# hjsuh94/irs_mpc

Measured on AMD Instinct MI355X. Metric: rollouts*timesteps/s (randomized-smoothing pass) + iLQR-iters/s, higher is better.
Workload: dtype f32; 1 GPU; planar_hand quasi-dynamic contact, zero-order-B smoothing, step QP solved exactly (dual active-set method) -- the metric's config; T=50, N_per_gpu=10000, N_total=10000, mode=ZERO_ORDER_B, contact_solver=exact, samples=supplied, resident in HBM (f32), parallelism=samples sharded over 1 GPU(s), 1 all-reduce of (T,P) f64 per step

## Files before the change

irs_mpc_amd/csrc/smooth_ug.hip:

```cpp
#include "smooth_common.hpp"

namespace {

#ifndef IRS_UG_SWEEPS
#define IRS_UG_SWEEPS 6
#endif
#ifndef IRS_UG_PDAS
#define IRS_UG_PDAS 4
#endif
#ifndef IRS_UG_BLOCK
#define IRS_UG_BLOCK 512
#endif
constexpr int kUgBlock = IRS_UG_BLOCK;
constexpr int kUgSweeps = IRS_UG_SWEEPS;
constexpr int kUgPdas = IRS_UG_PDAS;
#ifndef IRS_UG_STEP_COLUMNS
#define IRS_UG_STEP_COLUMNS 1
#endif
constexpr bool kUgStepColumns = IRS_UG_STEP_COLUMNS != 0;
constexpr int kUgTabH = 8, kUgTabTau = 40, kUgTabSet = 48, kUgTabX = 52;
constexpr int kUgTabStride = 116;
#ifndef IRS_UG_NOM_ROUNDS
#define IRS_UG_NOM_ROUNDS 2
#endif
constexpr int kUgNomRounds = IRS_UG_NOM_ROUNDS;
constexpr int kUgRing = 128;

template <class Model>
struct alignas(16) UgLds {
    static constexpr int NC = Model::NC, n = Model::NX, m = Model::NU;
    float tab[1 << NC][kUgTabStride];
    float W[NC][NC];
    float invw[NC];
    float Wd[NC];
    float r0[NC];
    float phi[NC];
    float C[m][NC];
    float JD[n][NC];
    float Jc[NC][n];
    float Dinv[n];
    float Db0[n];
    float DK[m];
    float q[n];
};

__device__ __forceinline__ float ug_uniform(float v) {
    return __int_as_float(__builtin_amdgcn_readfirstlane(__float_as_int(v)));
}

template <int NC>
struct UgUni {
    float W[NC * (NC + 1) / 2];
    float invw[NC];
    float r0[NC];
    __device__ __forceinline__ float w(int i, int j) const {
        return i <= j ? W[i * NC - i * (i - 1) / 2 + (j - i)] : W[j * NC - j * (j - 1) / 2 + (i - j)];
    }
};

template <class Model>
__device__ __forceinline__ unsigned ug_lookup_affine(const UgLds<Model>& S, unsigned a, const float* du, float tol,
                                                     float* v, float* tau) {
    constexpr int NC = Model::NC, m = Model::NU;
    static_assert(NC == 8 && m == 4, "table entries are 8 rows by 4 commands");
    const float4* e = reinterpret_cast<const float4*>(&S.tab[a][0]);
    float4 g4[kUgTabSet / 4];
#pragma unroll
    for (int c = 0; c < kUgTabSet / 4; ++c) g4[c] = e[c];
    const unsigned ap = __float_as_uint(S.tab[a][kUgTabSet]);
    tau[0] = g4[kUgTabTau / 4].x; tau[1] = g4[kUgTabTau / 4].y; tau[2] = g4[kUgTabTau / 4].z; tau[3] = g4[kUgTabTau / 4].w;
    tau[4] = g4[kUgTabTau / 4 + 1].x; tau[5] = g4[kUgTabTau / 4 + 1].y; tau[6] = g4[kUgTabTau / 4 + 1].z; tau[7] = g4[kUgTabTau / 4 + 1].w;
    v[0] = fmaf(tau[0], tol, g4[0].x); v[1] = fmaf(tau[1], tol, g4[0].y);
    v[2] = fmaf(tau[2], tol, g4[0].z); v[3] = fmaf(tau[3], tol, g4[0].w);
    v[4] = fmaf(tau[4], tol, g4[1].x); v[5] = fmaf(tau[5], tol, g4[1].y);
    v[6] = fmaf(tau[6], tol, g4[1].z); v[7] = fmaf(tau[7], tol, g4[1].w);
#pragma unroll
    for (int j = 0; j < m; ++j) {
        const float4 lo = g4[kUgTabH / 4 + 2 * j], hi = g4[kUgTabH / 4 + 2 * j + 1];
        v[0] = fmaf(lo.x, du[j], v[0]); v[1] = fmaf(lo.y, du[j], v[1]);
        v[2] = fmaf(lo.z, du[j], v[2]); v[3] = fmaf(lo.w, du[j], v[3]);
        v[4] = fmaf(hi.x, du[j], v[4]); v[5] = fmaf(hi.y, du[j], v[5]);
        v[6] = fmaf(hi.z, du[j], v[6]); v[7] = fmaf(hi.w, du[j], v[7]);
    }
    return ap;
}

template <class Model, bool UCOL>
__device__ __forceinline__ void ug_step_direction(const UgLds<Model>& S, unsigned a, int p, float* u, float* tau) {
    constexpr int NC = Model::NC;
    const float* e = &S.tab[a][0];
    const float4 t0 = *reinterpret_cast<const float4*>(e + kUgTabTau), t1 = *reinterpret_cast<const float4*>(e + kUgTabTau + 4);
    if constexpr (UCOL) {
        const float4 lo = *reinterpret_cast<const float4*>(e + kUgTabX + NC * p);
        const float4 hi = *reinterpret_cast<const float4*>(e + kUgTabX + NC * p + 4);
        u[0] = lo.x; u[1] = lo.y; u[2] = lo.z; u[3] = lo.w;
        u[4] = hi.x; u[5] = hi.y; u[6] = hi.z; u[7] = hi.w;
    } else {
        const float4 wlo = *reinterpret_cast<const float4*>(&S.W[p][0]);
        const float4 whi = *reinterpret_cast<const float4*>(&S.W[p][4]);
        const float4* x4 = reinterpret_cast<const float4*>(e + kUgTabX);
        float4 g4[2 * NC];
#pragma unroll
        for (int c = 0; c < 2 * NC; ++c) g4[c] = x4[c];
        const float wp[NC] = {wlo.x, wlo.y, wlo.z, wlo.w, whi.x, whi.y, whi.z, whi.w};
#pragma unroll
        for (int i = 0; i < NC; ++i) u[i] = 0.f;
#pragma unroll
        for (int c = 0; c < NC; ++c) {
            const float4 lo = g4[2 * c], hi = g4[2 * c + 1];
            u[0] = fmaf(lo.x, wp[c], u[0]); u[1] = fmaf(lo.y, wp[c], u[1]);
            u[2] = fmaf(lo.z, wp[c], u[2]); u[3] = fmaf(lo.w, wp[c], u[3]);
            u[4] = fmaf(hi.x, wp[c], u[4]); u[5] = fmaf(hi.y, wp[c], u[5]);
            u[6] = fmaf(hi.z, wp[c], u[6]); u[7] = fmaf(hi.w, wp[c], u[7]);
        }
    }
    tau[0] = t0.x; tau[1] = t0.y; tau[2] = t0.z; tau[3] = t0.w;
    tau[4] = t1.x; tau[5] = t1.y; tau[6] = t1.z; tau[7] = t1.w;
}

template <class Model>
__device__ __forceinline__ float ug_rhs(const UgUni<Model::NC>& U, const UgLds<Model>& S, const float* du, float* r) {
    constexpr int NC = Model::NC, m = Model::NU;
#pragma unroll
    for (int c = 0; c < NC; ++c) r[c] = U.r0[c];
#pragma unroll
    for (int j = 0; j < m; ++j) {
        const float4 lo = *reinterpret_cast<const float4*>(&S.C[j][0]);
        const float4 hi = *reinterpret_cast<const float4*>(&S.C[j][4]);
        r[0] = fmaf(lo.x, du[j], r[0]); r[1] = fmaf(lo.y, du[j], r[1]);
        r[2] = fmaf(lo.z, du[j], r[2]); r[3] = fmaf(lo.w, du[j], r[3]);
        r[4] = fmaf(hi.x, du[j], r[4]); r[5] = fmaf(hi.y, du[j], r[5]);
        r[6] = fmaf(hi.z, du[j], r[6]); r[7] = fmaf(hi.w, du[j], r[7]);
    }
    float scale = 1e-30f;
#pragma unroll
    for (int c = 0; c < NC; ++c) scale = fmaxf(scale, fabsf(r[c]));
    return 1e-6f * scale;
}

template <class Model>
__device__ __forceinline__ bool ug_try(const UgUni<Model::NC>& U, const UgLds<Model>& S, const float* r, const float* du,
                                       float tolv, float* lam, unsigned& a_out, int diag = 0) {
    constexpr int NC = Model::NC;
    float g[NC];
#pragma unroll
    for (int i = 0; i < NC; ++i) { lam[i] = 0.f; g[i] = r[i]; }
#pragma unroll 2
    for (int sw = 0; sw < ((diag & 64) ? 0 : kUgSweeps); ++sw) {
#pragma unroll
        for (int i = 0; i < NC; ++i) {
            const float nw = fmaxf(fmaf(-g[i], U.invw[i], lam[i]), 0.f);
            const float dl = nw - lam[i];
            lam[i] = nw;
#pragma unroll
            for (int j = 0; j < NC; ++j) g[j] = fmaf(U.w(j, i), dl, g[j]);
        }
    }
    unsigned a = 0u;
#pragma unroll
    for (int i = 0; i < NC; ++i) a |= (lam[i] > 0.f) ? (1u << i) : 0u;
    bool done = (diag & 32) != 0;
    for (int it = 0; it < kUgPdas; ++it) {
        float v[NC], tau[NC];
        const unsigned ap = ug_lookup_affine<Model>(S, a, du, tolv, v, tau);
        unsigned bad = 0u;
#pragma unroll
        for (int i = NC - 1; i >= 0; --i) bad = __builtin_amdgcn_alignbit(bad, __float_as_uint(v[i]), 31);
        if (!done) {
            if (bad == 0u) {
#pragma unroll
                for (int i = 0; i < NC; ++i) lam[i] = fmaf(-tau[i], v[i], v[i]);
                done = true;
            }
            a = ap ^ bad;
        }
        if (__all(done)) break;
    }
    a_out = a;
    return done;
}

template <class Model, bool UCOL>
__device__ __forceinline__ void ug_full(const UgLds<Model>& S, const float* r, const float* du, float tolv, unsigned a,
                                        float* lam, int cap = 4 * Model::NC) {
    constexpr int NC = Model::NC;
    constexpr float kBig = 3.0e38f, piv_rel = 1e-5f;
    float g[NC];
    bool valid = false;
    for (int round = 0; round < 3; ++round) {
        if (__all(valid)) break;
        float v[NC], tau[NC];
        const unsigned ap = ug_lookup_affine<Model>(S, a, du, 0.f, v, tau);
        if (!valid) {
            unsigned negb = 0u;
#pragma unroll
            for (int i = 0; i < NC; ++i) {
                const bool in = tau[i] == 0.f;
                negb |= (in && !(v[i] > 0.f)) ? (1u << i) : 0u;
                lam[i] = in ? v[i] : 0.f;
                g[i] = in ? 0.f : v[i];
            }
            valid = negb == 0u;
            a = ap & ~negb;
        }
    }
    if (!valid) {
        a = 0u;
#pragma unroll
        for (int i = 0; i < NC; ++i) { lam[i] = 0.f; g[i] = r[i]; }
    }
    int p = -1;
    bool done = false;
    for (int it = 0; it < cap; ++it) {
        if (!done && p < 0) {
            float vmin = kBig;
            int c = 0;
#pragma unroll
            for (int i = 0; i < NC; ++i) {
                const float vv = ((a >> i) & 1u) ? kBig : g[i];
                if (vv < vmin) { vmin = vv; c = i; }
            }
            if (vmin >= -tolv) done = true;
            else p = c;
        }
        if (__all(done)) break;
        const int pp = (done || p < 0) ? 0 : p;
        float u[NC], tau[NC];
        ug_step_direction<Model, UCOL>(S, a, pp, u, tau);
        const float wpp = S.Wd[pp];
        float gp = 0.f, zp = 0.f;
#pragma unroll
        for (int i = 0; i < NC; ++i) {
            const bool isp = i == pp;
            gp = isp ? g[i] : gp;
            zp = isp ? u[i] : zp;
        }
        const bool full_ok = zp > piv_rel * wpp;
        const float t2 = full_ok ? -gp * irs_rcp_fast(zp) : kBig;
        float rho[NC], qv[NC];
        float t1 = kBig;
#pragma unroll
        for (int i = 0; i < NC; ++i) {
            rho[i] = fmaf(tau[i], u[i], -u[i]);
            qv[i] = rho[i] > 0.f ? lam[i] * irs_rcp_fast(rho[i]) : kBig;
            t1 = fminf(t1, qv[i]);
        }
        int kb = 0;
#pragma unroll
        for (int i = NC - 1; i >= 0; --i) kb = (qv[i] == t1) ? i : kb;
        const float tmin = fminf(t1, t2);
        if (!done && !(tmin < kBig)) done = true;
        const float tt = done ? 0.f : tmin;
#pragma unroll
        for (int i = 0; i < NC; ++i) {
            g[i] = fmaf(tt * tau[i], u[i], g[i]);
            lam[i] = fmaxf(fmaf(-tt, rho[i], lam[i]) + ((i == pp) ? tt : 0.f), 0.f);
        }
        if (!done) {
            const bool full = t2 <= t1;
            if (full) {
                a |= 1u << pp;
                p = -1;
            } else {
                a &= ~(1u << kb);
#pragma unroll
                for (int i = 0; i < NC; ++i) lam[i] = (i == kb) ? 0.f : lam[i];
            }
        }
    }
}

template <class Model, bool UCOL>
__device__ __forceinline__ void ug_build_entry(UgLds<Model>& S, unsigned a, int half) {
    constexpr int NC = Model::NC;
    constexpr float piv_rel = 1e-5f;
    float M_[NC][NC], inv[NC], W[NC][NC];
    bool act[NC];
#pragma unroll
    for (int i = 0; i < NC; ++i) {
        act[i] = ((a >> i) & 1u) != 0u;
#pragma unroll
        for (int j = 0; j < NC; ++j) W[i][j] = S.W[i][j];
#pragma unroll
        for (int j = 0; j <= i; ++j) M_[i][j] = W[i][j];
    }
    unsigned ap = 0u;
#pragma unroll
    for (int j = 0; j < NC; ++j) {
        const float dj = M_[j][j];
        const bool ok = act[j] && dj > piv_rel * W[j][j];
        act[j] = ok;
        ap |= ok ? (1u << j) : 0u;
        inv[j] = ok ? irs_rcp_fast(dj) : 0.f;
#pragma unroll
        for (int i = j + 1; i < NC; ++i) M_[j][i] = M_[i][j] * inv[j];
#pragma unroll
        for (int i = j + 1; i < NC; ++i)
#pragma unroll
            for (int k = j + 1; k <= i; ++k) M_[i][k] = M_[i][k] - M_[j][i] * M_[k][j];
    }
    float* e = &S.tab[a][0];
    constexpr int NAPP = 1 + Model::NU + NC, SHARE = (NAPP + 1) / 2;
    for (int qq = 0; qq < SHARE; ++qq) {
        const int q = half * SHARE + qq;
        if (q >= NAPP) break;
        const int c = q - (1 + Model::NU);
        float x[NC];
        if (UCOL || c < 0) {
            const float* src = q == 0 ? &S.r0[0] : (c < 0 ? &S.C[q - 1][0] : &S.W[c][0]);
            const float4 lo = *reinterpret_cast<const float4*>(src), hi = *reinterpret_cast<const float4*>(src + 4);
            x[0] = lo.x; x[1] = lo.y; x[2] = lo.z; x[3] = lo.w;
            x[4] = hi.x; x[5] = hi.y; x[6] = hi.z; x[7] = hi.w;
        } else {
#pragma unroll
            for (int i = 0; i < NC; ++i) x[i] = (i == c) ? 1.f : 0.f;
        }
        float y[NC];
#pragma unroll
        for (int j = 0; j < NC; ++j) {
            float v = act[j] ? -x[j] : 0.f;
#pragma unroll
            for (int k = 0; k < j; ++k) v = v - M_[k][j] * y[k];
            y[j] = v;
        }
#pragma unroll
        for (int j = NC - 1; j >= 0; --j) {
            float v = y[j] * inv[j];
#pragma unroll
            for (int i = j + 1; i < NC; ++i) v = v - M_[j][i] * y[i];
            y[j] = v;
        }
        float col[NC];
#pragma unroll
        for (int i = 0; i < NC; ++i) {
            float s = x[i];
#pragma unroll
            for (int j = 0; j < NC; ++j) s = fmaf(W[i][j], y[j], s);
            col[i] = act[i] ? y[i] : s;
        }
        float* dst = e + (c < 0 ? NC * q : kUgTabX + NC * c);
        *reinterpret_cast<float4*>(dst) = make_float4(col[0], col[1], col[2], col[3]);
        *reinterpret_cast<float4*>(dst + 4) = make_float4(col[4], col[5], col[6], col[7]);
    }
    if (half == 1) {
        *reinterpret_cast<float4*>(e + kUgTabTau) = make_float4(act[0] ? 0.f : 1.f, act[1] ? 0.f : 1.f, act[2] ? 0.f : 1.f, act[3] ? 0.f : 1.f);
        *reinterpret_cast<float4*>(e + kUgTabTau + 4) = make_float4(act[4] ? 0.f : 1.f, act[5] ? 0.f : 1.f, act[6] ? 0.f : 1.f, act[7] ? 0.f : 1.f);
        e[kUgTabSet] = __uint_as_float(ap);
    }
}

struct UgNomLds {
    double J[8][7];
    double q[7], Dinv[7], b[7];
};

template <class Model, class Args>
__device__ __forceinline__ double ug_nominal_geometry(const Args& a, UgNomLds& L, int t, int lane) {
    constexpr int NC = Model::NC, n = Model::NX, m = Model::NU;
    double x64[n], u64[m], q[n], Dinv[n], b[n], J[NC][n], phi[NC];
#pragma unroll
    for (int i = 0; i < n; ++i) x64[i] = a.x_trj[(size_t)t * n + i];
#pragma unroll
    for (int j = 0; j < m; ++j) u64[j] = a.u_trj[(size_t)t * m + j];
    Model::template assemble<double>(a.p, x64, u64, q, Dinv, b, J, phi);
    if (lane == 0) {
#pragma unroll
        for (int c = 0; c < NC; ++c)
#pragma unroll
            for (int k = 0; k < n; ++k) L.J[c][k] = J[c][k];
#pragma unroll
        for (int k = 0; k < n; ++k) { L.q[k] = q[k]; L.Dinv[k] = Dinv[k]; L.b[k] = b[k]; }
    }
    double rr = 0.0;
#pragma unroll
    for (int c = 0; c < NC; ++c) {
        double s = phi[c];
#pragma unroll
        for (int k = 0; k < n; ++k) s -= J[c][k] * (b[k] * Dinv[k]);
        rr = (lane == c) ? s : rr;
    }
    wave_sync();
    return rr;
}

template <class Model, bool UCOL, class Args>
__device__ __forceinline__ void ug_nominal(const Args& a, const UgUni<Model::NC>& U, const UgLds<Model>& S,
                                           UgNomLds& L, double rr, int t, int lane) {
    constexpr int NC = Model::NC, n = Model::NX, m = Model::NU;
    static_assert(NC == 8 && n <= 8, "lane (i,k) = 8 i + k owns entry (i,k) of the 8 x 8 dual Hessian");
    float du0[m], r32[NC], lam32[NC];
#pragma unroll
    for (int j = 0; j < m; ++j) du0[j] = 0.f;
    const float tolv = ug_rhs<Model>(U, S, du0, r32);
    unsigned am = 0u;
    if (!ug_try<Model>(U, S, r32, du0, tolv, lam32, am)) ug_full<Model, UCOL>(S, r32, du0, tolv, am, lam32);
    unsigned set = 0u;
#pragma unroll
    for (int i = 0; i < NC; ++i) set |= (lam32[i] > 0.f) ? (1u << i) : 0u;
    set = (unsigned)__builtin_amdgcn_readfirstlane((int)set);
    {
        const int li = lane >> 3, lk = lane & 7;
        double w = 0.0;
#pragma unroll
        for (int kk = 0; kk < n; ++kk) w += L.J[li][kk] * L.Dinv[kk] * L.J[lk][kk];
        double scale = 1e-300;
#pragma unroll
        for (int c = 0; c < NC; ++c) scale = fmax(scale, fabs(__shfl(rr, c, 64)));
        const double tol64 = 1e-10 * scale;
        double lamd = 0.0;
        bool settled = false;
        for (int corr = 0; corr < 8 && !settled; ++corr) {
            double M = w, Lf = 0.0;
            unsigned eff = 0u;
            double invd[NC];
#pragma unroll
            for (int j = 0; j < NC; ++j) {
                const double dj = __shfl(M, 9 * j, 64), wjj = __shfl(w, 9 * j, 64);
                const bool ok = ((set >> j) & 1u) && dj > 1e-7 * wjj;
                eff |= ok ? (1u << j) : 0u;
                invd[j] = ok ? 1.0 / dj : 0.0;
                const double Mij = __shfl(M, 8 * li + j, 64), Mkj = __shfl(M, 8 * lk + j, 64);
                if (lk == j && li > j) Lf = Mij * invd[j];
                if (li > j && lk > j) M -= Mij * invd[j] * Mkj;
            }
            const bool mine = lane < NC && ((eff >> lane) & 1u);
            double y = mine ? -rr : 0.0;
#pragma unroll
            for (int j = 0; j < NC; ++j) {
                const double yj = __shfl(y, j, 64);
                const double Lij = __shfl(Lf, 8 * (lane & 7) + j, 64);
                if (lane < NC && lane > j) y -= Lij * yj;
            }
            double invme = 0.0;
#pragma unroll
            for (int j = 0; j < NC; ++j) invme = (lane == j) ? invd[j] : invme;
            y *= invme;
#pragma unroll
            for (int j = NC - 1; j >= 0; --j) {
                const double yj = __shfl(y, j, 64);
                const double Lji = __shfl(Lf, 8 * j + (lane & 7), 64);
                if (lane < j) y -= Lji * yj;
            }
            lamd = mine ? y : 0.0;
            double pr = w * __shfl(lamd, lk, 64);
            pr += __shfl_xor(pr, 1, 64);
            pr += __shfl_xor(pr, 2, 64);
            pr += __shfl_xor(pr, 4, 64);
            const double sl = rr + __shfl(pr, 8 * (lane & 7), 64);
            const bool neg = lane < NC && mine && !(lamd > 0.0);
            const bool viol = lane < NC && !mine && sl < -tol64;
            const unsigned negb = (unsigned)(__ballot(neg) & 0xffull), violb = (unsigned)(__ballot(viol) & 0xffull);
            if ((negb | violb) == 0u) settled = true;
            else set = (eff & ~negb) | violb;
        }
        double f = 0.0;
        if (settled) {
            double acc = 0.0;
#pragma unroll
            for (int c = 0; c < NC; ++c) acc += L.J[c][lane < n ? lane : 0] * __shfl(lamd, c, 64);
            if (lane < n) f = L.q[lane] + L.Dinv[lane] * (acc - L.b[lane]);
        } else if (lane < n) {
            float acc = -S.Db0[lane];
#pragma unroll
            for (int c = 0; c < NC; ++c) acc = fmaf(S.JD[lane][c], lam32[c], acc);
            f = (double)(S.q[lane] + acc);
        }
        if (lane < n)
            __hip_atomic_store(a.fnom + (size_t)t * n + Model::perm(lane), f, __ATOMIC_RELAXED, __HIP_MEMORY_SCOPE_AGENT);
    }
}

#ifdef IRS_UG_STAMPS
constexpr int kUgStampSlots = 12, kUgStampWgs = 2048;
__device__ unsigned long long ug_stamps[kUgStampWgs * kUgStampSlots];
#define UG_STAMP(slot)                                                                          \
    do {                                                                                        \
        if ((threadIdx.x & 63) == 0) {                                                          \
            const int wg_ = blockIdx.y * gridDim.x + blockIdx.x;                                \
            if (wg_ < kUgStampWgs && ((slot) < 8 ? threadIdx.x == 0 : true))                    \
                ug_stamps[wg_ * kUgStampSlots + (slot)] = __builtin_amdgcn_s_memtime();         \
        }                                                                                       \
    } while (0)
#else
#define UG_STAMP(slot) do {} while (0)
#endif

template <class Model, int MODE, bool RNG, bool FUSE, bool BATCH>
__global__ __launch_bounds__(kUgBlock) void smooth_ug_kernel(SmoothArgs args, std::conditional_t<BATCH, SmoothBatch, SmoothSolo> bat) {
    using TR = SmoothTraits<Model, MODE>;
    constexpr int n = TR::n, m = TR::m, P = TR::P, NC = Model::NC;
    constexpr int BLOCK = kUgBlock, NW = BLOCK / 64;
    static_assert(TR::Z0 == n && NC == 8 && m == 4, "u-only smoothing of an 8-row contact model with 4 commands");
    static_assert(P < kBlock, "the hand-off's group reduction");
    constexpr int NG = m * (m + 1) / 2;
    constexpr int PI = TR::FIRST_B ? 1 : NG + m * NC + m;
    constexpr int PPI = irs_reduce_pad(TR::FIRST_B ? n * m : PI);
    constexpr int QE = m + 1;
    constexpr bool UCOL = !TR::FIRST_B && kUgStepColumns;
    __shared__ UgLds<Model> S;
    __shared__ UgNomLds nomL;
    __shared__ float ring_all[NW * kUgRing * QE];
    __shared__ float red[NW * (PPI > TR::PP ? PPI : TR::PP)];
    __shared__ float toti[PPI];
    __shared__ unsigned hist[TR::FIRST_B ? (1 << NC) : 1];
    __shared__ double red64[TR::NGRP * P];
    __shared__ double tot[P];
    __shared__ FinalizeLds<Model, MODE> fin;
    __shared__ int s_ticket;

    decltype(auto) a = smooth_row<Model, MODE>(args, bat, (int)blockIdx.y);
    const int t = smooth_row_t(a, (int)blockIdx.y), blk = blockIdx.x, tid = threadIdx.x;
    const int lane = tid & 63, wave = tid >> 6;

    UG_STAMP(0);
    const bool nominal_wave = blk == 0 && wave == NW - 1;
    double nom_r = 0.0;
    if (nominal_wave && !(a.diag & 2)) nom_r = ug_nominal_geometry<Model>(a, nomL, t, lane);
    if (wave == 0) {
        float xb[n], ub[m], q[n], Dinv[n], b0[n], J[NC][n], phi[NC];
#pragma unroll
        for (int i = 0; i < n; ++i) xb[i] = (float)a.x_trj[(size_t)t * n + i];
#pragma unroll
        for (int j = 0; j < m; ++j) ub[j] = (float)a.u_trj[(size_t)t * m + j];
        Model::template assemble<float>(a.p, xb, ub, q, Dinv, b0, J, phi);
        if (lane == 0) {
#pragma unroll
            for (int i = 0; i < NC; ++i) {
                S.phi[i] = phi[i];
#pragma unroll
                for (int k = 0; k < n; ++k) S.Jc[i][k] = J[i][k];
            }
#pragma unroll
            for (int k = 0; k < n; ++k) { S.Db0[k] = b0[k] * Dinv[k]; S.q[k] = q[k]; S.Dinv[k] = Dinv[k]; }
#pragma unroll
            for (int j = 0; j < m; ++j) S.DK[j] = Dinv[Model::act(j)] * Model::template stiffness<float>(a.p, j);
        }
    }
    if constexpr (TR::FIRST_B) {
        for (int q = tid; q < (1 << NC); q += BLOCK) hist[q] = 0u;
    }
    __syncthreads();
    if (tid < NC * NC) {
        const int i = tid / NC, j = tid % NC, hi = i > j ? i : j, lo = i > j ? j : i;
        float w = (S.Jc[hi][0] * S.Dinv[0]) * S.Jc[lo][0];
#pragma unroll
        for (int k = 1; k < n; ++k) w = w + (S.Jc[hi][k] * S.Dinv[k]) * S.Jc[lo][k];
        S.W[i][j] = w;
        if (i == j) {
            S.Wd[i] = w;
            S.invw[i] = (float)kContactPgsOmega * irs_rcp_fast(w);
        }
    } else if (tid < NC * NC + NC) {
        const int i = tid - NC * NC;
        float ri = S.phi[i];
#pragma unroll
        for (int k = 0; k < n; ++k) ri = ri - S.Jc[i][k] * S.Db0[k];
        S.r0[i] = ri;
    } else if (tid < 2 * NC * NC + NC) {
        const int e = tid - (NC * NC + NC), k = e / NC, c = e % NC;
        if (k < n) S.JD[k][c] = S.Jc[c][k] * S.Dinv[k];
    } else if (tid < 2 * NC * NC + NC + m * NC) {
        const int e = tid - (2 * NC * NC + NC), j = e / NC, c = e % NC;
        S.C[j][c] = (S.Jc[c][Model::act(j)] * S.Dinv[Model::act(j)]) * Model::template stiffness<float>(a.p, j);
    }
    __syncthreads();
    UG_STAMP(1);
    if (!(a.diag & 4))
        for (int e = tid; e < 2 * (1 << NC); e += BLOCK) ug_build_entry<Model, UCOL>(S, (unsigned)(e >> 1), e & 1);
    __syncthreads();

    UG_STAMP(2);
    UgUni<NC> U;
    {
        int q = 0;
#pragma unroll
        for (int i = 0; i < NC; ++i)
#pragma unroll
            for (int j = i; j < NC; ++j) U.W[q++] = S.W[i][j];
#pragma unroll
        for (int i = 0; i < NC; ++i) { U.invw[i] = S.invw[i]; U.r0[i] = S.r0[i]; }
    }

    float acc[PPI];
#pragma unroll
    for (int i = 0; i < PPI; ++i) acc[i] = 0.f;

    if (nominal_wave && !(a.diag & 2)) ug_nominal<Model, UCOL>(a, U, S, nomL, nom_r, t, lane);
    if (nominal_wave) UG_STAMP(8);
    if (!(a.diag & 8)) {
        const int V = a.nblk * NW;
        const int me = nominal_wave ? V - 1 : (blk == 0 ? wave : blk * NW - 1 + wave);
        const int nblocks = (a.N + 63) / 64;
        int round = nominal_wave ? kUgNomRounds : 0;
        auto block_of = [&](int k) { return k < kUgNomRounds ? k * (V - 1) + me : kUgNomRounds * (V - 1) + (k - kUgNomRounds) * V + me; };
        float* ring = ring_all + wave * (kUgRing * QE);
        int qhead = 0, qtail = 0;
        int bk = block_of(round);
        float du_next[m];
#pragma unroll
        for (int j = 0; j < m; ++j) du_next[j] = 0.f;
        auto request = [&](int block) {
            if constexpr (!RNG) {
                if (block < nblocks) {
                    const int sidx = block * 64 + lane;
                    const size_t row = (size_t)t * a.N + (sidx < a.N ? sidx : a.N - 1);
                    load_row<m>(a.du + row * m, du_next);
                }
            }
        };
        request(bk);
        while (true) {
            const bool fresh = bk < nblocks;
            const int pending = qtail - qhead;
            const bool flush = pending >= 64 || (!fresh && pending > 0);
            if (!fresh && !flush) break;
            float du[m], r[NC], lam[NC];
            bool on, fin_ = true;
            if (flush) {
                __builtin_amdgcn_fence(__ATOMIC_RELEASE, "wavefront");
                __builtin_amdgcn_wave_barrier();
                __builtin_amdgcn_fence(__ATOMIC_ACQUIRE, "wavefront");
                const int take = min(64, pending);
                on = lane < take;
                const int slot = (qhead + (on ? lane : 0)) & (kUgRing - 1);
#pragma unroll
                for (int j = 0; j < m; ++j) du[j] = ring[slot * QE + j];
                const unsigned wm = __float_as_uint(ring[slot * QE + m]);
                const float tolv = ug_rhs<Model>(U, S, du, r);
                ug_full<Model, UCOL>(S, r, du, tolv, wm, lam, (a.diag & 128) ? 8 : ((a.diag & 256) ? 12 : 4 * NC));
                qhead += take;
            } else {
                const int sidx = bk * 64 + lane;
                on = sidx < a.N;
                if constexpr (RNG) {
                    const unsigned long long gidx = a.sample_offset + (unsigned long long)sidx;
#pragma unroll
                    for (int j = n / 4; j < (n + m + 3) / 4; ++j) {
                        float g4[4];
                        philox_normal4(gidx, (unsigned)t, (unsigned)j, a.iter, a.seed, g4);
#pragma unroll
                        for (int c = 0; c < 4; ++c) {
                            const int idx = 4 * j + c;
                            if (idx >= n && idx < n + m) du[idx - n] = __fmul_rn(g4[c], a.std[idx]);
                        }
                    }
                } else {
#pragma unroll
                    for (int j = 0; j < m; ++j) du[j] = du_next[j];
                    request(block_of(round + 1));
                }
                const float tolv = ug_rhs<Model>(U, S, du, r);
                unsigned mask = 0u;
                fin_ = ug_try<Model>(U, S, r, du, tolv, lam, mask, a.diag);
                if (a.diag & 16) fin_ = true;
                const bool hard = on && !fin_;
                const unsigned long long bal = __ballot(hard);
                if (hard) {
                    const int slot = (qtail + __popcll(bal & ((1ull << lane) - 1ull))) & (kUgRing - 1);
#pragma unroll
                    for (int j = 0; j < m; ++j) ring[slot * QE + j] = du[j];
                    ring[slot * QE + m] = __uint_as_float(mask);
                }
                qtail += __popcll(bal);
                bk = block_of(++round);
            }
            const bool use = on && fin_;
            bool nonfinite = false;
#pragma unroll
            for (int j = 0; j < m; ++j) nonfinite = nonfinite || irs_nonfinite_bits(du[j]);
            if constexpr (TR::FIRST_B) {
                unsigned I = 0u;
#pragma unroll
                for (int i = 0; i < NC; ++i) I |= (lam[i] * S.Wd[i] > (float)kContactActiveTol) ? (1u << i) : 0u;
                if (use) __hip_atomic_fetch_add(&hist[I], 1u, __ATOMIC_RELAXED, __HIP_MEMORY_SCOPE_WORKGROUP);
                if (on && nonfinite) acc[0] = irs_poison();
            } else {
                float zz[m];
#pragma unroll
                for (int j = 0; j < m; ++j) zz[j] = use ? du[j] : 0.f;
                int q = 0;
#pragma unroll
                for (int i = 0; i < m; ++i)
#pragma unroll
                    for (int j = i; j < m; ++j) { acc[q] = fmaf(zz[i], zz[j], acc[q]); ++q; }
#pragma unroll
                for (int i = 0; i < m; ++i)
#pragma unroll
                    for (int c = 0; c < NC; ++c) { acc[q] = fmaf(zz[i], lam[c], acc[q]); ++q; }
#pragma unroll
                for (int i = 0; i < m; ++i) { acc[q] += zz[i]; ++q; }
                if (on && nonfinite) acc[0] = irs_poison();
            }
        }
    }

    UG_STAMP(3);
    if (blk == 0 && wave == 1) UG_STAMP(9);
    if constexpr (TR::FIRST_B) {
        __syncthreads();
        unsigned poison_bits = __float_as_uint(acc[0]);
        asm volatile("" : "+v"(poison_bits));
#pragma unroll
        for (int i = 0; i < PPI; ++i) acc[i] = 0.f;
        for (int I = tid; I < (1 << NC); I += BLOCK) {
            const unsigned cnt = hist[I];
            if (cnt == 0u) continue;
            const float* e = &S.tab[I][0];
            const unsigned ap = __float_as_uint(e[kUgTabSet]);
            float Y[NC][m];
#pragma unroll
            for (int i = 0; i < NC; ++i) {
                const bool in = ((ap >> i) & 1u) != 0u;
#pragma unroll
                for (int c = 0; c < m; ++c) {
                    float s = 0.f;
#pragma unroll
                    for (int j = 0; j < NC; ++j) s = fmaf(e[kUgTabX + 8 * j + i], S.Jc[j][Model::act(c)], s);
                    Y[i][c] = in ? -s : 0.f;
                }
            }
#pragma unroll
            for (int k = 0; k < n; ++k)
#pragma unroll
                for (int c = 0; c < m; ++c) {
                    float s = 0.f;
#pragma unroll
                    for (int i = 0; i < NC; ++i) s = fmaf(S.Jc[i][k], Y[i][c], s);
                    const float Bkc = (k == Model::act(c) ? 1.f : 0.f) - S.Dinv[k] * s;
                    acc[Model::perm(k) * m + c] += (float)cnt * Bkc;
                }
        }
        if ((poison_bits & 0x7f800000u) == 0x7f800000u) acc[0] = irs_poison();
        block_reduce_lds<P, NW>(acc, red);
    } else {
        block_reduce_lds<PI, NW>(acc, red);
        __syncthreads();
        for (int q = tid; q < PI; q += BLOCK) {
            float s = red[q];
#pragma unroll
            for (int w = 1; w < NW; ++w) s += red[w * PPI + q];
            toti[q] = s;
        }
        __syncthreads();
        float out = 0.f;
        if (tid < P) {
            if (tid < NG) out = toti[tid];
            else if (tid < NG + m * n) {
                const int i = (tid - NG) / n, kext = (tid - NG) % n;
                int k = 0, jact = -1;
#pragma unroll
                for (int kk = 0; kk < n; ++kk) k = (Model::perm(kk) == kext) ? kk : k;
#pragma unroll
                for (int j = 0; j < m; ++j) jact = (Model::act(j) == k) ? j : jact;
                float s = -S.Db0[k] * toti[NG + m * NC + i];
                for (int c = 0; c < NC; ++c) s = fmaf(S.JD[k][c], toti[NG + i * NC + c], s);
                if (jact >= 0) {
                    const int lo = i < jact ? i : jact, hi = i < jact ? jact : i;
                    s = fmaf(S.DK[jact], toti[lo * m - lo * (lo - 1) / 2 + (hi - lo)], s);
                }
                out = s;
            } else {
                out = toti[NG + m * NC + (tid - NG - m * n)];
            }
        }
        __syncthreads();
        for (int q = tid; q < NW * TR::PP; q += BLOCK) red[q] = 0.f;
        __syncthreads();
        if (tid < P) red[tid] = out;
    }
    UG_STAMP(4);
    smooth_finish<Model, MODE, FUSE, BLOCK, true, std::remove_cv_t<std::remove_reference_t<decltype(a)>>>(a, red, red64, tot, fin, s_ticket, t, blk, tid, a.fnom + (size_t)t * n);
    UG_STAMP(5);
}

template <class Model, int MODE>
void ug_launch_m(const SmoothArgs& a, bool rng, bool fuse, hipStream_t st) {
    dim3 grid(a.nblk, a.T), block(kUgBlock);
    if (rng) {
        if (fuse) hipLaunchKernelGGL((smooth_ug_kernel<Model, MODE, true, true, false>), grid, block, 0, st, a, SmoothSolo{});
        else hipLaunchKernelGGL((smooth_ug_kernel<Model, MODE, true, false, false>), grid, block, 0, st, a, SmoothSolo{});
    } else {
        if (fuse) hipLaunchKernelGGL((smooth_ug_kernel<Model, MODE, false, true, false>), grid, block, 0, st, a, SmoothSolo{});
        else hipLaunchKernelGGL((smooth_ug_kernel<Model, MODE, false, false, false>), grid, block, 0, st, a, SmoothSolo{});
    }
}

template <class Model, int MODE>
void ug_launch_batch_m(const SmoothArgs& a, const SmoothBatch& bat, int B, hipStream_t st) {
    dim3 grid(a.nblk, B * a.T), block(kUgBlock);
    hipLaunchKernelGGL((smooth_ug_kernel<Model, MODE, true, true, true>), grid, block, 0, st, a, bat);
}

}

#ifdef IRS_UG_STAMPS
extern "C" int irs_debug_ug_stamps(unsigned long long* host_out, int n_wgs) {
    if (n_wgs > kUgStampWgs) n_wgs = kUgStampWgs;
    return (int)hipMemcpyFromSymbol(host_out, HIP_SYMBOL(ug_stamps), (size_t)n_wgs * kUgStampSlots * sizeof(unsigned long long));
}
#endif

bool irs_smooth_ug_supported(int model, int mode) {
    const char* e = getenv("IRS_UG");
    if (e != nullptr && atoi(e) == 0) return false;
    return model == IRS_MODEL_PLANAR_HAND_EXACT && (mode == IRS_SMOOTH_ZERO_ORDER_B || mode == IRS_SMOOTH_FIRST_ORDER);
}

int irs_smooth_ug_nblk(int T, int N) {
    static int cus = 0;
    if (cus == 0) {
        hipDeviceProp_t prop;
        int dev = 0;
        cus = (hipGetDevice(&dev) == hipSuccess && hipGetDeviceProperties(&prop, dev) == hipSuccess)
                  ? prop.multiProcessorCount : 256;
        if (cus < 1) cus = 256;
    }
    const int nblocks = (N + 63) / 64, NW = kUgBlock / 64;
    int nb = cus / (T < 1 ? 1 : T);
    if (nb < 1) nb = 1;
    const int by_work = (nblocks + 1 + NW - 1) / NW;
    if (nb > by_work) nb = by_work;
    return nb < 1 ? 1 : nb;
}

int irs_smooth_ug_launch(int model, int mode, const SmoothArgs& a, bool rng, bool fuse, hipStream_t st) {
    if (model != IRS_MODEL_PLANAR_HAND_EXACT) return IRS_ERR_UNSUPPORTED;
    if (mode == IRS_SMOOTH_ZERO_ORDER_B) ug_launch_m<PlanarHandExactModel, IRS_SMOOTH_ZERO_ORDER_B>(a, rng, fuse, st);
    else if (mode == IRS_SMOOTH_FIRST_ORDER) ug_launch_m<PlanarHandExactModel, IRS_SMOOTH_FIRST_ORDER>(a, rng, fuse, st);
    else return IRS_ERR_UNSUPPORTED;
    return IRS_OK;
}

int irs_smooth_ug_launch_batch(int model, int mode, const SmoothArgs& a, const SmoothBatch& bat, int B, hipStream_t st) {
    if (model != IRS_MODEL_PLANAR_HAND_EXACT) return IRS_ERR_UNSUPPORTED;
    if (mode == IRS_SMOOTH_ZERO_ORDER_B) ug_launch_batch_m<PlanarHandExactModel, IRS_SMOOTH_ZERO_ORDER_B>(a, bat, B, st);
    else if (mode == IRS_SMOOTH_FIRST_ORDER) ug_launch_batch_m<PlanarHandExactModel, IRS_SMOOTH_FIRST_ORDER>(a, bat, B, st);
    else return IRS_ERR_UNSUPPORTED;
    return IRS_OK;
}
```

Measured before the change: 13.93 billion rollouts*timesteps/s.

## Build active-set table by shared-prefix principal pivoting across lane groups

Replaces the per-entry table build, which solved each of the 256 active-set subsystems independently, with a tableau pivoting scheme. Eight lanes hold one tableau and use ds_swizzle broadcasts, and subsets share pivot prefixes so the last two pivots fan out into four entries. The goal is to cut redundant arithmetic in the per-workgroup prologue. It also moves the prologue into a shared helper and adds a debug kernel that dumps the table, while keeping the old LDL path behind a macro; differences in pivot order and the pivot threshold can change numerics slightly.

```diff
diff --git a/irs_mpc_amd/csrc/smooth_ug.hip b/irs_mpc_amd/csrc/smooth_ug.hip
--- a/irs_mpc_amd/csrc/smooth_ug.hip
+++ b/irs_mpc_amd/csrc/smooth_ug.hip
@@ -18,6 +18,10 @@
 #define IRS_UG_STEP_COLUMNS 1
 #endif
 constexpr bool kUgStepColumns = IRS_UG_STEP_COLUMNS != 0;
+#ifndef IRS_UG_TABLE_LDL
+#define IRS_UG_TABLE_LDL 0
+#endif
+constexpr bool kUgTableLdl = IRS_UG_TABLE_LDL != 0;
 constexpr int kUgTabH = 8, kUgTabTau = 40, kUgTabSet = 48, kUgTabX = 52;
 constexpr int kUgTabStride = 116;
 #ifndef IRS_UG_NOM_ROUNDS
@@ -349,6 +353,101 @@
     }
 }
 
+template <int NS>
+struct UgTableau {
+    float c[NS][8];
+    unsigned set;
+};
+
+template <int P>
+__device__ __forceinline__ float ug_bcast8(float v) {
+    return __int_as_float(__builtin_amdgcn_ds_swizzle(__float_as_int(v), 0x18 | (P << 5)));
+}
+
+template <int P, int NS>
+__device__ __forceinline__ void ug_pivot(UgTableau<NS>& R, bool want, float wpp) {
+    constexpr float piv_rel = 1e-5f;
+    constexpr int PS = (5 + P) >> 3, PL = (5 + P) & 7;
+    float x[8];
+#pragma unroll
+    for (int i = 0; i < 8; ++i) x[i] = ug_bcast8<PL>(R.c[PS][i]);
+    const float d = x[P];
+    const bool ok = want && d > piv_rel * wpp;
+    const float rinv = ok ? -irs_rcp_fast(d) : 0.f;
+#pragma unroll
+    for (int s = 0; s < NS; ++s) {
+        const float rho = R.c[s][P] * rinv;
+#pragma unroll
+        for (int i = 0; i < 8; ++i)
+            if (i != P) R.c[s][i] = fmaf(x[i], rho, R.c[s][i]);
+        R.c[s][P] = ok ? rho : R.c[s][P];
+    }
+    R.set |= ok ? (1u << P) : 0u;
+}
+
+template <class Model, bool UCOL, int NS>
+__device__ __forceinline__ void ug_emit_entry(UgLds<Model>& S, unsigned a, const UgTableau<NS>& R, int l) {
+    float* e = &S.tab[a][0];
+    auto put = [&](int off, const float* v) {
+        *reinterpret_cast<float4*>(e + off) = make_float4(v[0], v[1], v[2], v[3]);
+        *reinterpret_cast<float4*>(e + off + 4) = make_float4(v[4], v[5], v[6], v[7]);
+    };
+    if constexpr (UCOL) put(l < 5 ? 8 * l : kUgTabX + 8 * (l - 5), R.c[0]);
+    else put(kUgTabX + 8 * l, R.c[2]);
+    const float* v = UCOL ? R.c[1] : R.c[0];
+    const int half = l == 6 ? 4 : 0;
+    float4 q;
+    q.x = l < 5 ? v[0] : (l == 7 ? __uint_as_float(R.set) : (((R.set >> (half + 0)) & 1u) ? 0.f : 1.f));
+    q.y = l < 5 ? v[1] : (l == 7 ? 0.f : (((R.set >> (half + 1)) & 1u) ? 0.f : 1.f));
+    q.z = l < 5 ? v[2] : (l == 7 ? 0.f : (((R.set >> (half + 2)) & 1u) ? 0.f : 1.f));
+    q.w = l < 5 ? v[3] : (l == 7 ? 0.f : (((R.set >> (half + 3)) & 1u) ? 0.f : 1.f));
+    const int off = l < 5 ? (UCOL ? kUgTabX + 8 * (l + 3) : 8 * l) : (l == 7 ? kUgTabSet : kUgTabTau + half);
+    *reinterpret_cast<float4*>(e + off) = q;
+    if (l < 5) *reinterpret_cast<float4*>(e + off + 4) = make_float4(v[4], v[5], v[6], v[7]);
+}
+
+template <class Model, bool UCOL>
+__device__ __forceinline__ void ug_build_table(UgLds<Model>& S, int tid) {
+    constexpr int NC = Model::NC, NS = UCOL ? 2 : 3, NW = kUgBlock / 64;
+    static_assert(NC == 8 && Model::NU == 4, "an 8 x 13 tableau, eight lanes each");
+    const int l = tid & 7;
+    for (int w = __builtin_amdgcn_readfirstlane(tid >> 6); w < 8; w += NW) {
+        const unsigned shared = (unsigned)(w ^ ((w & 4) ? 3 : 0));
+        const unsigned g = ((unsigned)(tid >> 3) & 7u) | (shared << 3);
+        UgTableau<NS> R;
+        {
+            const float* c0 = l == 0 ? &S.r0[0] : (l < 5 ? &S.C[l - 1][0] : &S.W[l - 5][0]);
+            const float* c1 = &S.W[l < 5 ? l + 3 : 0][0];
+            const float4 a0 = *reinterpret_cast<const float4*>(c0), a1 = *reinterpret_cast<const float4*>(c0 + 4);
+            const float4 b0 = *reinterpret_cast<const float4*>(c1), b1 = *reinterpret_cast<const float4*>(c1 + 4);
+            R.c[0][0] = a0.x; R.c[0][1] = a0.y; R.c[0][2] = a0.z; R.c[0][3] = a0.w;
+            R.c[0][4] = a1.x; R.c[0][5] = a1.y; R.c[0][6] = a1.z; R.c[0][7] = a1.w;
+            R.c[1][0] = b0.x; R.c[1][1] = b0.y; R.c[1][2] = b0.z; R.c[1][3] = b0.w;
+            R.c[1][4] = b1.x; R.c[1][5] = b1.y; R.c[1][6] = b1.z; R.c[1][7] = b1.w;
+            if constexpr (!UCOL) {
+#pragma unroll
+                for (int i = 0; i < NC; ++i) R.c[2][i] = (l == i) ? 1.f : 0.f;
+            }
+        }
+        R.set = 0u;
+        ug_pivot<0>(R, (g & 1u) != 0u, S.Wd[0]);
+        ug_pivot<1>(R, (g & 2u) != 0u, S.Wd[1]);
+        ug_pivot<2>(R, (g & 4u) != 0u, S.Wd[2]);
+        if (shared & 1u) ug_pivot<3>(R, true, S.Wd[3]);
+        if (shared & 2u) ug_pivot<4>(R, true, S.Wd[4]);
+        if (shared & 4u) ug_pivot<5>(R, true, S.Wd[5]);
+        UgTableau<NS> R6 = R, R7 = R;
+        ug_pivot<6>(R6, true, S.Wd[6]);
+        ug_pivot<7>(R7, true, S.Wd[7]);
+        UgTableau<NS> R67 = R6;
+        ug_pivot<7>(R67, true, S.Wd[7]);
+        ug_emit_entry<Model, UCOL>(S, g, R, l);
+        ug_emit_entry<Model, UCOL>(S, g | 64u, R6, l);
+        ug_emit_entry<Model, UCOL>(S, g | 128u, R7, l);
+        ug_emit_entry<Model, UCOL>(S, g | 192u, R67, l);
+    }
+}
+
 struct UgNomLds {
     double J[8][7];
     double q[7], Dinv[7], b[7];
@@ -484,6 +583,79 @@
 #else
 #define UG_STAMP(slot) do {} while (0)
 #endif
+
+template <class Model, bool UCOL>
+__device__ __forceinline__ void ug_prologue(const ModelParams& p, const double* x, const double* u, bool build,
+                                            UgLds<Model>& S, int tid) {
+    constexpr int n = Model::NX, m = Model::NU, NC = Model::NC;
+    const int lane = tid & 63, wave = tid >> 6;
+    if (wave == 0) {
+        float xb[n], ub[m], q[n], Dinv[n], b0[n], J[NC][n], phi[NC];
+#pragma unroll
+        for (int i = 0; i < n; ++i) xb[i] = (float)x[i];
+#pragma unroll
+        for (int j = 0; j < m; ++j) ub[j] = (float)u[j];
+        Model::template assemble<float>(p, xb, ub, q, Dinv, b0, J, phi);
+        if (lane == 0) {
+#pragma unroll
+            for (int i = 0; i < NC; ++i) {
+                S.phi[i] = phi[i];
+#pragma unroll
+                for (int k = 0; k < n; ++k) S.Jc[i][k] = J[i][k];
+            }
+#pragma unroll
+            for (int k = 0; k < n; ++k) { S.Db0[k] = b0[k] * Dinv[k]; S.q[k] = q[k]; S.Dinv[k] = Dinv[k]; }
+#pragma unroll
+            for (int j = 0; j < m; ++j) S.DK[j] = Dinv[Model::act(j)] * Model::template stiffness<float>(p, j);
+        }
+    }
+    __syncthreads();
+    if (tid < NC * NC) {
+        const int i = tid / NC, j = tid % NC, hi = i > j ? i : j, lo = i > j ? j : i;
+        float w = (S.Jc[hi][0] * S.Dinv[0]) * S.Jc[lo][0];
+#pragma unroll
+        for (int k = 1; k < n; ++k) w = w + (S.Jc[hi][k] * S.Dinv[k]) * S.Jc[lo][k];
+        S.W[i][j] = w;
+        if (i == j) {
+            S.Wd[i] = w;
+            S.invw[i] = (float)kContactPgsOmega * irs_rcp_fast(w);
+        }
+    } else if (tid < NC * NC + NC) {
+        const int i = tid - NC * NC;
+        float ri = S.phi[i];
+#pragma unroll
+        for (int k = 0; k < n; ++k) ri = ri - S.Jc[i][k] * S.Db0[k];
+        S.r0[i] = ri;
+    } else if (tid < 2 * NC * NC + NC) {
+        const int e = tid - (NC * NC + NC), k = e / NC, c = e % NC;
+        if (k < n) S.JD[k][c] = S.Jc[c][k] * S.Dinv[k];
+    } else if (tid < 2 * NC * NC + NC + m * NC) {
+        const int e = tid - (2 * NC * NC + NC), j = e / NC, c = e % NC;
+        S.C[j][c] = (S.Jc[c][Model::act(j)] * S.Dinv[Model::act(j)]) * Model::template stiffness<float>(p, j);
+    }
+    __syncthreads();
+    UG_STAMP(1);
+    if (build) {
+        if constexpr (kUgTableLdl) {
+            for (int e = tid; e < 2 * (1 << NC); e += kUgBlock) ug_build_entry<Model, UCOL>(S, (unsigned)(e >> 1), e & 1);
+        } else {
+            ug_build_table<Model, UCOL>(S, tid);
+        }
+    }
+    __syncthreads();
+}
+
+template <class Model, bool UCOL>
+__global__ __launch_bounds__(kUgBlock) void ug_table_kernel(ModelParams p, const double* x, const double* u, float* out) {
+    __shared__ UgLds<Model> S;
+    const int tid = threadIdx.x;
+    ug_prologue<Model, UCOL>(p, x, u, true, S, tid);
+    constexpr int NE = 1 << Model::NC;
+    for (int q = tid; q < NE * kUgTabStride; q += kUgBlock) {
+        const int c = q % kUgTabStride;
+        out[q] = (c > kUgTabSet && c < kUgTabX) ? 0.f : S.tab[q / kUgTabStride][c];
+    }
+}
 
 template <class Model, int MODE, bool RNG, bool FUSE, bool BATCH>
 __global__ __launch_bounds__(kUgBlock) void smooth_ug_kernel(SmoothArgs args, std::conditional_t<BATCH, SmoothBatch, SmoothSolo> bat) {
@@ -516,58 +688,10 @@
     const bool nominal_wave = blk == 0 && wave == NW - 1;
     double nom_r = 0.0;
     if (nominal_wave && !(a.diag & 2)) nom_r = ug_nominal_geometry<Model>(a, nomL, t, lane);
-    if (wave == 0) {
-        float xb[n], ub[m], q[n], Dinv[n], b0[n], J[NC][n], phi[NC];
-#pragma unroll
-        for (int i = 0; i < n; ++i) xb[i] = (float)a.x_trj[(size_t)t * n + i];
-#pragma unroll
-        for (int j = 0; j < m; ++j) ub[j] = (float)a.u_trj[(size_t)t * m + j];
-        Model::template assemble<float>(a.p, xb, ub, q, Dinv, b0, J, phi);
-        if (lane == 0) {
-#pragma unroll
-            for (int i = 0; i < NC; ++i) {
-                S.phi[i] = phi[i];
-#pragma unroll
-                for (int k = 0; k < n; ++k) S.Jc[i][k] = J[i][k];
-            }
-#pragma unroll
-            for (int k = 0; k < n; ++k) { S.Db0[k] = b0[k] * Dinv[k]; S.q[k] = q[k]; S.Dinv[k] = Dinv[k]; }
-#pragma unroll
-            for (int j = 0; j < m; ++j) S.DK[j] = Dinv[Model::act(j)] * Model::template stiffness<float>(a.p, j);
-        }
-    }
     if constexpr (TR::FIRST_B) {
         for (int q = tid; q < (1 << NC); q += BLOCK) hist[q] = 0u;
     }
-    __syncthreads();
-    if (tid < NC * NC) {
-        const int i = tid / NC, j = tid % NC, hi = i > j ? i : j, lo = i > j ? j : i;
-        float w = (S.Jc[hi][0] * S.Dinv[0]) * S.Jc[lo][0];
-#pragma unroll
-        for (int k = 1; k < n; ++k) w = w + (S.Jc[hi][k] * S.Dinv[k]) * S.Jc[lo][k];
-        S.W[i][j] = w;
-        if (i == j) {
-            S.Wd[i] = w;
-            S.invw[i] = (float)kContactPgsOmega * irs_rcp_fast(w);
-        }
-    } else if (tid < NC * NC + NC) {
-        const int i = tid - NC * NC;
-        float ri = S.phi[i];
-#pragma unroll
-        for (int k = 0; k < n; ++k) ri = ri - S.Jc[i][k] * S.Db0[k];
-        S.r0[i] = ri;
-    } else if (tid < 2 * NC * NC + NC) {
-        const int e = tid - (NC * NC + NC), k = e / NC, c = e % NC;
-        if (k < n) S.JD[k][c] = S.Jc[c][k] * S.Dinv[k];
-    } else if (tid < 2 * NC * NC + NC + m * NC) {
-        const int e = tid - (2 * NC * NC + NC), j = e / NC, c = e % NC;
-        S.C[j][c] = (S.Jc[c][Model::act(j)] * S.Dinv[Model::act(j)]) * Model::template stiffness<float>(a.p, j);
-    }
-    __syncthreads();
-    UG_STAMP(1);
-    if (!(a.diag & 4))
-        for (int e = tid; e < 2 * (1 << NC); e += BLOCK) ug_build_entry<Model, UCOL>(S, (unsigned)(e >> 1), e & 1);
-    __syncthreads();
+    ug_prologue<Model, UCOL>(a.p, a.x_trj + (size_t)t * n, a.u_trj + (size_t)t * m, !(a.diag & 4), S, tid);
 
     UG_STAMP(2);
     UgUni<NC> U;
@@ -800,6 +924,32 @@
 }
 #endif
 
+extern "C" int irs_debug_ug_table(int model, const double* params, const double* x, const double* u, int first_order,
+                                  float* out_256x116) {
+    using Model = PlanarHandExactModel;
+    if (model != IRS_MODEL_PLANAR_HAND_EXACT) return IRS_ERR_UNSUPPORTED;
+    IRS_CHECK_ARG(x && u && out_256x116, "null pointer");
+    ModelParams p;
+    int rc = irs_load_params(model, params, Model::NPARAMS, &p);
+    if (rc != IRS_OK) return rc;
+    constexpr size_t NOUT = (size_t)(1 << Model::NC) * kUgTabStride;
+    double* dxu = nullptr;
+    float* dout = nullptr;
+    if (hipMalloc(&dxu, (Model::NX + Model::NU) * sizeof(double)) != hipSuccess) return IRS_ERR_HIP;
+    if (hipMalloc(&dout, NOUT * sizeof(float)) != hipSuccess) { (void)hipFree(dxu); return IRS_ERR_HIP; }
+    hipError_t e = hipMemcpy(dxu, x, Model::NX * sizeof(double), hipMemcpyHostToDevice);
+    if (e == hipSuccess) e = hipMemcpy(dxu + Model::NX, u, Model::NU * sizeof(double), hipMemcpyHostToDevice);
+    if (e == hipSuccess) {
+        if (first_order) hipLaunchKernelGGL((ug_table_kernel<Model, false>), dim3(1), dim3(kUgBlock), 0, 0, p, dxu, dxu + Model::NX, dout);
+        else hipLaunchKernelGGL((ug_table_kernel<Model, kUgStepColumns>), dim3(1), dim3(kUgBlock), 0, 0, p, dxu, dxu + Model::NX, dout);
+        e = hipGetLastError();
+    }
+    if (e == hipSuccess) e = hipMemcpy(out_256x116, dout, NOUT * sizeof(float), hipMemcpyDeviceToHost);
+    (void)hipFree(dxu);
+    (void)hipFree(dout);
+    return e == hipSuccess ? IRS_OK : IRS_ERR_HIP;
+}
+
 bool irs_smooth_ug_supported(int model, int mode) {
     const char* e = getenv("IRS_UG");
     if (e != nullptr && atoi(e) == 0) return false;
```

Measured after the change: 14.64 billion rollouts*timesteps/s, median of 6. 5.1% higher.
